# BUTSpeechFIT/DiariZen

Measured on AMD Instinct MI355X. Metric: audio-seconds/s (RTF) for wavlm-large-s80 pipeline, 16 kHz mono, higher is better.
Workload: dtype f32 (operands split into 2 fp16 terms with exact power-of-two scaling = 22 significant bits, 3 fp16 MFMA products, fp32 accumulate: the error-corrected '3xFP16/3xTF32' scheme; kernels without an fp16 variant use the 3-term bf16 split)

## Files before the change

### diarizen_amd/csrc/gemm.hip

```cpp
#include <cstdio>
#include <cstdlib>

#include "common.h"
#include "gemm_epilogue.h"

namespace {

template <bool LOWP>
struct Frag {
  using type = f32x4;
};
template <>
struct Frag<true> {
  using type = bf16x8;
};

__device__ __forceinline__ uint4 pack_bf16x8(const float4& a, const float4& b) {
  bf16x8 v;
  v[0] = (__bf16)a.x; v[1] = (__bf16)a.y; v[2] = (__bf16)a.z; v[3] = (__bf16)a.w;
  v[4] = (__bf16)b.x; v[5] = (__bf16)b.y; v[6] = (__bf16)b.z; v[7] = (__bf16)b.w;
  return *reinterpret_cast<uint4*>(&v);
}

template <int BM, int BN, int WGM, int WGN, bool LOWP>
// ... 88 lines not shown
        rw[i] = make_uint4(0u, 0u, 0u, 0u);
      }
    }
  };

  auto store_tile = [&](int buf) {
    unsigned char* sA = smem + buf * BUF;
    unsigned char* sW = sA + BM * 128;
#pragma unroll
    for (int i = 0; i < ACH; ++i) {
      const int r = r0 + 32 * i;
      const int off = r * 128 + ((c ^ ((r >> 1) & 7)) << 4);
      if constexpr (LOWP)
        *reinterpret_cast<uint4*>(sA + off) = pack_bf16x8(ra[i][0], ra[i][1]);
      else
        *reinterpret_cast<float4*>(sA + off) = ra[i][0];
    }
#pragma unroll
    for (int i = 0; i < WCH; ++i) {
      const int r = r0 + 32 * i;
      const int off = r * 128 + ((c ^ ((r >> 1) & 7)) << 4);
      *reinterpret_cast<uint4*>(sW + off) = rw[i];
    }
  };

  f32x4 acc[MI][NI];
#pragma unroll
  for (int i = 0; i < MI; ++i)
#pragma unroll
    for (int j = 0; j < NI; ++j) acc[i][j] = (f32x4){0.f, 0.f, 0.f, 0.f};

  const int lr = lane & 15;
  const int lq = lane >> 4;

  auto compute = [&](int buf) {
    const unsigned char* sA = smem + buf * BUF;
    const unsigned char* sW = sA + BM * 128;
#pragma unroll
    for (int kb = 0; kb < 2; ++kb) {
      frag_t af[MI], bf[NI];
#pragma unroll
      for (int i = 0; i < MI; ++i) {
        const int row = wm * TM + i * 16 + lr;
        const int slot = (kb * 4 + lq) ^ ((row >> 1) & 7);
        af[i] = *reinterpret_cast<const frag_t*>(sA + row * 128 + (slot << 4));
      }
#pragma unroll
      for (int j = 0; j < NI; ++j) {
        const int row = wn * TN + j * 16 + lr;
        const int slot = (kb * 4 + lq) ^ ((row >> 1) & 7);
        bf[j] = *reinterpret_cast<const frag_t*>(sW + row * 128 + (slot << 4));
      }
      if constexpr (LOWP) {
#pragma unroll
        for (int i = 0; i < MI; ++i)
#pragma unroll
          for (int j = 0; j < NI; ++j)
            acc[i][j] = __builtin_amdgcn_mfma_f32_16x16x32_bf16(bf[j], af[i], acc[i][j], 0, 0, 0);
      } else {
#pragma unroll
        for (int s = 0; s < 4; ++s)
#pragma unroll
          for (int i = 0; i < MI; ++i)
#pragma unroll
            for (int j = 0; j < NI; ++j)
              acc[i][j] = __builtin_amdgcn_mfma_f32_16x16x4f32(bf[j][s], af[i][s], acc[i][j], 0, 0, 0);
      }
    }
  };

  const int nk = (d.K + BK - 1) / BK;
  load_tile(0);
  store_tile(0);
  __syncthreads();
  for (int kt = 0; kt < nk; ++kt) {
    const bool more = kt + 1 < nk;
    if (more) load_tile((kt + 1) * BK);
    compute(kt & 1);
    if (more) store_tile((kt + 1) & 1);
    __syncthreads();
  }

  gemm_epilogue<BM, BN, TM, TN, MI, NI>(d, acc, tm, tn, wm, wn, lr, lq, cz, bz, z0);
}

template <int BM, int BN, int WGM, int WGN>
__global__ __launch_bounds__(256) void gemm_glds_kernel(const dzn_gemm_desc d) {
  static_assert(WGM * WGN == 4, "4 wavefronts per workgroup");
  constexpr int BK = 32;
  constexpr int TM = BM / WGM, TN = BN / WGN;
  constexpr int MI = TM / 16, NI = TN / 16;
  constexpr int ACH = BM / 32, WCH = BN / 32;
  constexpr int BUF = (BM + BN) * 128;
  extern __shared__ __attribute__((aligned(16))) unsigned char smem[];

  const int tid = threadIdx.x, lane = tid & 63, wave = tid >> 6;
  const int wm = wave / WGN, wn = wave % WGN;
  const int tilesN = (d.N + BN - 1) / BN;
  int t;
  {
    const int nwg = gridDim.x, bid = blockIdx.x;
    const int q = nwg >> 3, r = nwg & 7, xcd = bid & 7, idx = bid >> 3;
    t = (xcd < r ? xcd * (q + 1) : r * (q + 1) + (xcd - r) * q) + idx;
  }
  const int tm = t / tilesN, tn = t % tilesN;
  const int z = blockIdx.y;
  int z0 = z / d.zdiv;
  const int z1 = z - z0 * d.zdiv;
  if (d.z_list) {
    if (z0 >= d.z_count[0]) return;
    z0 = d.z_list[z0];
  }
  const float* __restrict__ A = d.A + z0 * d.a_z0 + z1 * d.a_z1;
  const float* __restrict__ W = d.W + z0 * d.w_z0 + z1 * d.w_z1;
  const int64_t cz = z0 * d.c_z0 + z1 * d.c_z1;
  const int64_t bz = z0 * d.b_z0 + z1 * d.b_z1;

  const int r0 = tid >> 3;
  const int csw = (tid & 7) ^ ((r0 >> 1) & 7);
  int64_t abase[ACH], wbase[WCH];
#pragma unroll
  for (int i = 0; i < ACH; ++i) {
    int m = tm * BM + r0 + 32 * i;
    m = m < d.M ? m : d.M - 1;
    abase[i] = (d.a_rowoff ? (int64_t)d.a_rowoff[m] : (int64_t)m * d.lda) + csw * 4;
  }
#pragma unroll
  for (int i = 0; i < WCH; ++i) {
    int n = tn * BN + r0 + 32 * i;
    n = n < d.N ? n : d.N - 1;
    wbase[i] = (int64_t)n * d.ldw + csw * 4;
  }

  auto issue = [&](int k0, int buf) {
    const int ch = k0 / d.kc;
    const int64_t koff = (int64_t)ch * d.ldk + (k0 - ch * d.kc);
    unsigned char* sA = smem + buf * BUF + wave * 1024;
    unsigned char* sW = smem + buf * BUF + BM * 128 + wave * 1024;
#pragma unroll
    for (int i = 0; i < ACH; ++i)
      __builtin_amdgcn_global_load_lds(
          (const __attribute__((address_space(1))) void*)(A + abase[i] + koff),
          (__attribute__((address_space(3))) void*)(sA + i * 4096), 16, 0, 0);
#pragma unroll
    for (int i = 0; i < WCH; ++i)
      __builtin_amdgcn_global_load_lds(
          (const __attribute__((address_space(1))) void*)(W + wbase[i] + k0),
          (__attribute__((address_space(3))) void*)(sW + i * 4096), 16, 0, 0);
  };

  f32x4 acc[MI][NI];
#pragma unroll
  for (int i = 0; i < MI; ++i)
#pragma unroll
    for (int j = 0; j < NI; ++j) acc[i][j] = (f32x4){0.f, 0.f, 0.f, 0.f};
  const int lr = lane & 15, lq = lane >> 4;

  auto read_frags = [&](int buf, int kb, f32x4 (&af)[MI], f32x4 (&bf)[NI]) {
    const unsigned char* sA = smem + buf * BUF;
    const unsigned char* sW = sA + BM * 128;
#pragma unroll
    for (int i = 0; i < MI; ++i) {
      const int row = wm * TM + i * 16 + lr;
      const int slot = (kb * 4 + lq) ^ ((row >> 1) & 7);
      af[i] = *reinterpret_cast<const f32x4*>(sA + row * 128 + (slot << 4));
    }
#pragma unroll
    for (int j = 0; j < NI; ++j) {
      const int row = wn * TN + j * 16 + lr;
      const int slot = (kb * 4 + lq) ^ ((row >> 1) & 7);
      bf[j] = *reinterpret_cast<const f32x4*>(sW + row * 128 + (slot << 4));
    }
  };
  auto mma = [&](const f32x4 (&af)[MI], const f32x4 (&bf)[NI]) {
#pragma unroll
    for (int s = 0; s < 4; ++s)
#pragma unroll
      for (int i = 0; i < MI; ++i)
#pragma unroll
        for (int j = 0; j < NI; ++j)
          acc[i][j] = __builtin_amdgcn_mfma_f32_16x16x4f32(bf[j][s], af[i][s], acc[i][j], 0, 0, 0);
  };

  const int nk = d.K / BK;
  f32x4 a0[MI], b0[NI], a1[MI], b1[NI];
  issue(0, 0);
  __syncthreads();
  read_frags(0, 0, a0, b0);
  for (int kt = 0; kt < nk; ++kt) {
    const int buf = kt & 1;
    const bool more = kt + 1 < nk;
    if (more) issue((kt + 1) * BK, buf ^ 1);
    read_frags(buf, 1, a1, b1);
    __builtin_amdgcn_sched_barrier(0);
    mma(a0, b0);
    __builtin_amdgcn_sched_barrier(0);
    __syncthreads();
    if (more) read_frags(buf ^ 1, 0, a0, b0);
    __builtin_amdgcn_sched_barrier(0);
    mma(a1, b1);
    __builtin_amdgcn_sched_barrier(0);
  }
  gemm_epilogue<BM, BN, TM, TN, MI, NI>(d, acc, tm, tn, wm, wn, lr, lq, cz, bz, z0);
}

template <int BM, int BN, int WGM, int WGN, bool LOWP>
int launch_cfg(const dzn_gemm_desc& d, hipStream_t s) {
  const int tilesM = (d.M + BM - 1) / BM, tilesN = (d.N + BN - 1) / BN;
  static const int lds_pad = getenv("DZN_GEMM_LDS_PAD") ? atoi(getenv("DZN_GEMM_LDS_PAD")) : 0;
  const size_t lds = 2 * (BM + BN) * 128 + lds_pad;
  auto kern = gemm_kernel<BM, BN, WGM, WGN, LOWP>;
  static unsigned long long attr_mask = 0;
  if (first_use_on_device(attr_mask)) {
    (void)hipFuncSetAttribute(reinterpret_cast<const void*>(kern),
                        hipFuncAttributeMaxDynamicSharedMemorySize, 160 * 1024);
    if constexpr (!LOWP)
      (void)hipFuncSetAttribute(reinterpret_cast<const void*>(gemm_glds_kernel<BM, BN, WGM, WGN>),
                                hipFuncAttributeMaxDynamicSharedMemorySize, 160 * 1024);
  }
  static const bool no_glds = getenv("DZN_NO_GLDS") != nullptr;
  const bool use_glds = !LOWP && !no_glds && (d.K % 32 == 0) && (d.kc % 32 == 0);
  dim3 grid(tilesM * tilesN, d.nz > 0 ? d.nz : 1, 1);
  int pid = -1;
  if (prof_enabled()) {
    char cls[64];
    static const bool by_shape = getenv("DZN_PROFILE_SHAPES") != nullptr;
    if (by_shape)
      snprintf(cls, sizeof(cls), "gemm_%s_%dx%d M%d N%d K%d z%d", LOWP ? "bf16" : "f32", BM, BN, d.M, d.N,
               d.K, d.nz);
    else
      snprintf(cls, sizeof(cls), "gemm_%s_%dx%d", LOWP ? "bf16" : "f32", BM, BN);
    const double fl = d.alg_flops > 0 ? d.alg_flops * d.nz : 2.0 * d.M * d.N * d.K * d.nz;
    pid = prof_begin(s, cls, fl, gemm_alg_bytes(d, LOWP ? 2 : 4));
  }
  if constexpr (!LOWP) {
    if (use_glds)
      hipLaunchKernelGGL((gemm_glds_kernel<BM, BN, WGM, WGN>), grid, dim3(256), lds, s, d);
    else
      hipLaunchKernelGGL(kern, grid, dim3(256), lds, s, d);
  } else {
    hipLaunchKernelGGL(kern, grid, dim3(256), lds, s, d);
  }
  prof_end(pid, s);
  if (hipGetLastError() != hipSuccess) return DZN_E_HIP;
  if (d.stat_partial && d.stat_final)
    return launch_stats_finalize(d.stat_partial, d.M, ((d.N + BN - 1) / BN) * WGN, d.stat_C, d.stat_eps, d.stat_final, s);
  return DZN_OK;
}

template <bool LOWP>
int launch_prec(const dzn_gemm_desc& d, hipStream_t s) {
  static const char* force = getenv("DZN_GEMM_CFG");
  if (force) {
    if (!strcmp(force, "128x32")) return launch_cfg<128, 32, 4, 1, LOWP>(d, s);
    if (!strcmp(force, "256x32")) return launch_cfg<256, 32, 4, 1, LOWP>(d, s);
    if (!strcmp(force, "256x64")) return launch_cfg<256, 64, 4, 1, LOWP>(d, s);
    if (!strcmp(force, "128x64")) return launch_cfg<128, 64, 2, 2, LOWP>(d, s);
    if (!strcmp(force, "64x64")) return launch_cfg<64, 64, 2, 2, LOWP>(d, s);
    if (!strcmp(force, "128x128")) return launch_cfg<128, 128, 2, 2, LOWP>(d, s);
  }
  if (d.N <= 32) return launch_cfg<256, 32, 4, 1, LOWP>(d, s);
  if (d.N <= 64) return launch_cfg<128, 64, 2, 2, LOWP>(d, s);
  if (d.K <= 512 && (d.N % 64) == 0) return launch_cfg<128, 64, 2, 2, LOWP>(d, s);
  const int cand[4] = {192, 160, 128, 96};
  int best = 128, best_cols = 1 << 30;
  for (int c : cand) {
    const int cols = (d.N + c - 1) / c * c;
    if (cols < best_cols) { best_cols = cols; best = c; }
  }
  switch (best) {
    case 192: return launch_cfg<128, 192, 2, 2, LOWP>(d, s);
    case 160: return launch_cfg<128, 160, 2, 2, LOWP>(d, s);
    case 96: return launch_cfg<128, 96, 2, 2, LOWP>(d, s);
    default: return launch_cfg<128, 128, 2, 2, LOWP>(d, s);
  }
}

}

int launch_gemm(const dzn_gemm_desc& din, hipStream_t s) {
  dzn_gemm_desc d = din;
  if (d.M <= 0 || d.N <= 0) return DZN_OK;
  if (d.K <= 0 || (d.K & 7)) return DZN_E_INVALID;
  if (d.kc <= 0) { d.kc = d.K; d.ldk = 0; }
  if (d.kc & 7) return DZN_E_INVALID;
  if (d.zdiv <= 0) d.zdiv = 1;
  if (d.nz <= 0) d.nz = 1;
  if (d.alpha == 0.f) d.alpha = 1.f;
  if (d.precision == DZN_PREC_BF16) {
    if (!d.W16) return DZN_E_INVALID;
#ifdef DZN_TUNING
    if (d.a_bf16) return launch_gemm_lowp(d, s);
#else
    if (d.a_bf16) return DZN_E_INVALID;
#endif
    if (d.c_bf16 || d.r_bf16) return DZN_E_INVALID;
    return launch_prec<true>(d, s);
  }
  if (!d.W) return DZN_E_INVALID;
  if (d.kv_planes) {
    const bool ok = d.kv_scale && d.precision == DZN_PREC_F32_H2 && d.W3 && d.W2h && d.col_scale && d.a_amax && !(d.K & 31) &&
                    !(d.kc & 31) && d.ldw == d.K && !d.a_split3 && d.nz == 1 && !d.c_rowoff && d.kv_col0 >= 0 &&
                    d.kv_col0 < d.N && !(d.kv_col0 & 63) && !(d.N & 63) && d.kv_ld == d.N - d.kv_col0 &&
                    !(d.kv_plane_stride & 3) && d.N > 32 && !getenv("DZN_GEMM_CFG") && !getenv("DZN_NO_H2");
    if (!ok) return DZN_E_INVALID;
  }
  if (d.ln_centered && !(d.precision == DZN_PREC_F16 && d.W3 && !(d.K & 31) && !(d.kc & 31) && d.ldw == d.K && !d.a_split3))
    return DZN_E_INVALID;
  if (d.a_split3) return prec_is_split(d.precision) ? launch_gemm_split_pre(d, s) : DZN_E_INVALID;
  if (prec_is_split(d.precision) && d.W3 && !(d.K & 31) && !(d.kc & 31) && d.ldw == d.K)
    return launch_gemm_split(d, s);
  return launch_prec<false>(d, s);
}

extern "C" int dzn_op_gemm(const dzn_gemm_desc* d, void* stream) {
  if (!d || !d->A || !d->C) return DZN_E_INVALID;
  return launch_gemm(*d, reinterpret_cast<hipStream_t>(stream));
}
```

### diarizen_amd/csrc/gemm_split.hip

```cpp
#include <cmath>
#include <cstdio>
#include <cstdlib>
#include <type_traits>

#include "checked.h"
#include "common.h"
#include "gemm_epilogue.h"
#include "split.h"

DZN_CHECKED_TU(gemm_split)

namespace {

__device__ __forceinline__ int wswz(int row) { return (0x78 >> (2 * ((row >> 2) & 3))) & 3; }

template <int N>
__device__ __forceinline__ void wait_vm_lgkm0() {
  static_assert(N >= 0 && N < 64, "vmcnt range");
  __builtin_amdgcn_s_waitcnt((N & 0xF) | ((N >> 4) << 14) | (0x7 << 4));
}

template <int BM, int BN, int WGM, int WGN, int S, int NP, int OCC = 1, int ABL = 0, bool RPF = false>
__global__ __launch_bounds__(WGM * WGN * 64, OCC) void gemm_split_kernel(const dzn_gemm_desc d, const int ngroups) {
  constexpr int NW = WGM * WGN;
  constexpr int BK = 32;
  constexpr int TM = BM / WGM, TN = BN / WGN;
  constexpr int MI = TM / 16, NI = TN / 16, MH = MI / 2;
  constexpr int RB = NW * 1024;
  constexpr int ACH = BM * 128 / RB;
  constexpr int WROWS = NW * 16;
  constexpr int WR = (BN + WROWS - 1) / WROWS;
  constexpr int SP = NP == 3 ? 3 : 2;
  constexpr int ABYTES = BM * 128, WPLANE = BN * 64, BUF = ABYTES + NP * WPLANE;
  constexpr int LPT = ACH + NP * WR;
  constexpr bool WPART = BN % WROWS != 0;
  static_assert(BM * 128 % RB == 0, "A tile must be whole rounds");
  static_assert(MI % 2 == 0, "two row halves per wavefront tile");
  static_assert(S >= 2 && (S - 1) * LPT < 64, "vmcnt range");
  extern __shared__ __attribute__((aligned(16))) unsigned char smem[];

  const int tid = threadIdx.x, lane = tid & 63;
  const int wave = __builtin_amdgcn_readfirstlane(tid >> 6);
  const int wm = wave / WGN, wn = wave % WGN;
  const int tilesN = (d.N + BN - 1) / BN;
  int t;
  {
    const int nwg = gridDim.x, bid = blockIdx.x;
    const int q = nwg >> 3, r = nwg & 7, xcd = bid & 7, idx = bid >> 3;
    t = (xcd < r ? xcd * (q + 1) : r * (q + 1) + (xcd - r) * q) + idx;
  }
  int tm, tn;
  if (ngroups <= 1) {
    tm = t / tilesN;
    tn = t % tilesN;
  } else {
    const int tilesM_ = (int)gridDim.x / tilesN;
    const int base = tilesN / ngroups, rem = tilesN % ngroups;
    int g = 0, cg = base + (rem > 0), cs = 0, r = t;
    while (r >= tilesM_ * cg) {
      r -= tilesM_ * cg;
      cs += cg;
      ++g;
      cg = base + (g < rem);
    }
    tm = r / cg;
    tn = cs + r - tm * cg;
  }
  const int z = blockIdx.y;
  int z0 = z / d.zdiv;
  const int z1 = z - z0 * d.zdiv;
  if (d.z_list) {
    if (z0 >= d.z_count[0]) return;
    z0 = d.z_list[z0];
  }
  const float* __restrict__ A = d.A + z0 * d.a_z0 + z1 * d.a_z1;
  const u16* __restrict__ W3 =
      reinterpret_cast<const u16*>(NP == 3 ? d.W3 : d.W2h) + SP * (z0 * d.w_z0 + z1 * d.w_z1);
  float a_scale[MI], row_inv[MI];
#pragma unroll
  for (int i = 0; i < MI; ++i) a_scale[i] = row_inv[i] = 1.f;
  if constexpr (NP <= 2) {
#pragma unroll
    for (int i = 0; i < MI; ++i) {
      int m = tm * BM + wm * TM + i * 16 + (lane & 15);
      m = m < d.M ? m : d.M - 1;
      const int unit = d.amax_unit > 0 ? m / d.amax_unit : z0;
      DZN_CHECK(d.amax_count <= 0 || (unit >= 0 && unit < d.amax_count), 0x101, unit);
      h2_scale(d.a_amax[unit], a_scale[i], row_inv[i]);
    }
  }
  float a_mean[MI];
#pragma unroll
  for (int i = 0; i < MI; ++i) a_mean[i] = 0.f;
  if constexpr (NP == 1) {
    if (d.ln_centered && d.ln_stats) {
#pragma unroll
      for (int i = 0; i < MI; ++i) {
        int m = tm * BM + wm * TM + i * 16 + (lane & 15);
        m = m < d.M ? m : d.M - 1;
        a_mean[i] = d.ln_stats[2 * (int64_t)m];
        a_scale[i] *= 0.5f;
        row_inv[i] *= 2.f;
      }
    }
  }
  const int64_t cz = z0 * d.c_z0 + z1 * d.c_z1;
  const int64_t bz = z0 * d.b_z0 + z1 * d.b_z1;

  const int r0 = tid >> 3;
  const int csw = (tid & 7) ^ ((r0 >> 1) & 7);
  const float* aptr[ACH];
#pragma unroll
  for (int i = 0; i < ACH; ++i) {
    int m = tm * BM + r0 + 8 * NW * i;
    m = m < d.M ? m : d.M - 1;
    aptr[i] = A + (d.a_rowoff ? (int64_t)d.a_rowoff[m] : (int64_t)m * d.lda) + csw * 4;
  }
  const bool wfull = !WPART || (WR - 1) * WROWS + wave * 16 < BN;
  const int wr0 = wave * 16 + (lane >> 2);
  const int wsw = (lane & 3) ^ wswz(wr0);
  const u16* wptr[WR];
#pragma unroll
  for (int i = 0; i < WR; ++i) {
    int n = tn * BN + wr0 + WROWS * i;
    n = n < d.N ? n : d.N - 1;
    wptr[i] = W3 + (int64_t)n * SP * d.ldw + wsw * 8;
  }

  int ik = 0, irem = 0;
  int64_t ikoff = 0;
  auto issue = [&](int stage) {
    unsigned char* sA = smem + stage * BUF + wave * 1024;
    unsigned char* sW = smem + stage * BUF + ABYTES + wave * 1024;
    DZN_CHECK(stage >= 0 && stage < S && ik < d.K, 0x102, stage);
    DZN_CHECK(wave * 1024 + (ACH - 1) * RB + 1024 <= ABYTES, 0x103, wave);
    DZN_CHECK(!wfull || wave * 1024 + (WR - 1) * RB + 1024 <= WPLANE, 0x104, wave);
#pragma unroll
    for (int i = 0; i < ACH; ++i)
      __builtin_amdgcn_global_load_lds((const __attribute__((address_space(1))) void*)(aptr[i] + ikoff),
                                       (__attribute__((address_space(3))) void*)(sA + i * RB), 16, 0, 0);
#pragma unroll
    for (int p = 0; p < NP; ++p)
#pragma unroll
      for (int i = 0; i < WR; ++i)
        if (i + 1 < WR || wfull)
          __builtin_amdgcn_global_load_lds(
              (const __attribute__((address_space(1))) void*)(wptr[i] + SP * ik + p * 32),
              (__attribute__((address_space(3))) void*)(sW + p * WPLANE + i * RB), 16, 0, 0);
    ik += BK;
    irem += BK;
    ikoff += BK;
    if (irem == d.kc) { irem = 0; ikoff += d.ldk - d.kc; }
  };

  f32x4 acc[MI][NI];
#pragma unroll
  for (int i = 0; i < MI; ++i)
#pragma unroll
    for (int j = 0; j < NI; ++j) acc[i][j] = (f32x4){0.f, 0.f, 0.f, 0.f};
  const int lr = lane & 15, lq = lane >> 4;
  f32x4 rpre[RPF ? MI : 1][RPF ? NI : 1];
  bool use_rpre = false;
  if constexpr (RPF) {
    use_rpre = d.R != nullptr && gemm_epilogue_vec(d, cz, bz);
    if (use_rpre) gemm_prefetch_residual<BM, BN, TM, TN, MI, NI>(d, rpre, tm, tn, wm, wn, lr, lq, cz);
  }

  int woff[NI], aoff0[MI], aoff1[MI];
#pragma unroll
  for (int j = 0; j < NI; ++j) {
    const int row = wn * TN + j * 16 + lr;
    woff[j] = ABYTES + row * 64 + ((lq ^ wswz(row)) << 4);
  }
#pragma unroll
  for (int i = 0; i < MI; ++i) {
    const int row = wm * TM + i * 16 + lr;
    const int sw = (row >> 1) & 7;
    aoff0[i] = row * 128 + ((lq ^ sw) << 4);
    aoff1[i] = row * 128 + (((4 + lq) ^ sw) << 4);
  }
#pragma unroll
  for (int j = 0; j < NI; ++j) DZN_CHECK(woff[j] >= ABYTES && woff[j] + (NP - 1) * WPLANE + 16 <= BUF, 0x105, woff[j]);
#pragma unroll
  for (int i = 0; i < MI; ++i) DZN_CHECK(aoff0[i] + 16 <= ABYTES && aoff1[i] + 16 <= ABYTES, 0x106, aoff1[i]);
  DZN_CHECK(tm * BM < d.M && tn * BN < d.N, 0x107, t);
  auto read_w = [&](int stage, u32x4 (&wf)[NI][NP]) {
    const unsigned char* base = smem + stage * BUF;
#pragma unroll
    for (int j = 0; j < NI; ++j)
#pragma unroll
      for (int p = 0; p < NP; ++p) wf[j][p] = *reinterpret_cast<const u32x4*>(base + p * WPLANE + woff[j]);
  };
  auto read_a = [&](int stage, f32x4 (&ar)[MI][2]) {
    const unsigned char* base = smem + stage * BUF;
#pragma unroll
    for (int i = 0; i < MI; ++i) {
      ar[i][0] = *reinterpret_cast<const f32x4*>(base + aoff0[i]);
      ar[i][1] = *reinterpret_cast<const f32x4*>(base + aoff1[i]);
    }
  };
  auto mma = [&](int i, const u32x4 (&wf)[NI][NP], const u32x4 (&af)[NP]) {
    if constexpr (ABL == 2) {
#pragma unroll
      for (int j = 0; j < NI; ++j) acc[i][j][0] += __uint_as_float(wf[j][0][0] ^ af[0][0]);
    } else if constexpr (NP == 3) {
      constexpr int PW[6] = {2, 0, 1, 1, 0, 0}, PA[6] = {0, 2, 1, 0, 1, 0};
#pragma unroll
      for (int t = 0; t < 6; ++t)
#pragma unroll
        for (int j = 0; j < NI; ++j) acc[i][j] = mfma_np<NP>(wf[j][PW[t]], af[PA[t]], acc[i][j]);
    } else if constexpr (NP == 2) {
      constexpr int PW[3] = {1, 0, 0}, PA[3] = {0, 1, 0};
#pragma unroll
      for (int t = 0; t < 3; ++t)
#pragma unroll
        for (int j = 0; j < NI; ++j) acc[i][j] = mfma_np<NP>(wf[j][PW[t]], af[PA[t]], acc[i][j]);
    } else {
#pragma unroll
      for (int j = 0; j < NI; ++j) acc[i][j] = mfma_np<NP>(wf[j][0], af[0], acc[i][j]);
    }
  };
  auto split = [&](const f32x4 (&a)[2], u32x4 (&af)[NP], float sc, float mu = 0.f) {
    if constexpr (ABL == 1) {
#pragma unroll
      for (int p = 0; p < NP; ++p) af[p] = __builtin_bit_cast(u32x4, a[p & 1]);
    } else if constexpr (NP == 3) {
      bf16x8 h_, m_, l_;
      split8(a[0], a[1], h_, m_, l_);
      af[0] = __builtin_bit_cast(u32x4, h_);
      af[1] = __builtin_bit_cast(u32x4, m_);
      af[2] = __builtin_bit_cast(u32x4, l_);
    } else if constexpr (NP == 2) {
      split8_h2(a[0], a[1], sc, af[0], af[1]);
    } else {
      cvt8_h1(a[0] - mu, a[1] - mu, sc, af[0]);
    }
  };

  const int nk = d.K / BK;
#pragma unroll
  for (int s = 0; s < S; ++s)
    if (s < nk) issue(s);
  auto wait_tiles = [&](auto tiles) {
    constexpr int T = decltype(tiles)::value;
    if (wfull) wait_vm_lgkm0<T * LPT>();
    else wait_vm_lgkm0<T * (LPT - NP)>();
  };
  if (nk >= S) wait_tiles(std::integral_constant<int, S - 1>{});
  else wait_vm_lgkm0<0>();
  __builtin_amdgcn_s_barrier();
  u32x4 wfa[NI][NP], wfb[NI][NP];
  f32x4 ar[MI][2];
  read_w(0, wfa);
  read_a(0, ar);
  if constexpr (ABL == 5) read_w(0, wfb);
  int stage = 0;

  auto step = [&](int kt, const u32x4 (&wc)[NI][NP], u32x4 (&wn_)[NI][NP]) {
    const bool more = kt + 1 < nk;
#pragma unroll
    for (int i = 0; i < MH; ++i) {
      u32x4 af[NP];
      split(ar[i], af, a_scale[i], a_mean[i]);
      mma(i, wc, af);
    }
    u32x4 af2[MI - MH][NP];
#pragma unroll
    for (int i = MH; i < MI; ++i) split(ar[i], af2[i - MH], a_scale[i], a_mean[i]);
    const int nstage = stage + 1 == S ? 0 : stage + 1;
    __builtin_amdgcn_sched_barrier(0);
    if (more) {
      if (kt + S <= nk) wait_tiles(std::integral_constant<int, S - 2>{});
      else wait_vm_lgkm0<0>();
      if constexpr (ABL != 4) __builtin_amdgcn_s_barrier();
      if constexpr (ABL != 3)
        if (kt + S < nk) issue(stage);
      if constexpr (ABL != 5) {
        read_w(nstage, wn_);
        read_a(nstage, ar);
      }
    }
    __builtin_amdgcn_sched_barrier(0);
#pragma unroll
    for (int i = MH; i < MI; ++i) mma(i, wc, af2[i - MH]);
    stage = nstage;
  };
  for (int kt = 0; kt < nk; kt += 2) {
    step(kt, wfa, wfb);
    if (kt + 1 < nk) step(kt + 1, wfb, wfa);
  }
  if constexpr (true) {
    __syncthreads();
    if constexpr (RPF) {
      if (use_rpre) {
        gemm_epilogue<BM, BN, TM, TN, MI, NI, true>(d, acc, tm, tn, wm, wn, lr, lq, cz, bz, z0, row_inv, NP <= 2 ? d.col_scale : nullptr,
                                                    reinterpret_cast<float*>(smem) + wave * 3 * TN, rpre);
        return;
      }
    }
    gemm_epilogue<BM, BN, TM, TN, MI, NI, true>(d, acc, tm, tn, wm, wn, lr, lq, cz, bz, z0, row_inv, NP <= 2 ? d.col_scale : nullptr,
                                                reinterpret_cast<float*>(smem) + wave * 3 * TN);
  } else {
    gemm_epilogue<BM, BN, TM, TN, MI, NI>(d, acc, tm, tn, wm, wn, lr, lq, cz, bz, z0, row_inv, NP <= 2 ? d.col_scale : nullptr);
  }
}

#ifdef DZN_TUNING
typedef float f32x16 __attribute__((ext_vector_type(16)));

template <int BM, int BN, int WGM, int WGN, int S, int NP, int OCC = 1, int PRIO = 0>
__global__ __launch_bounds__(WGM * WGN * 64, OCC) void gemm_split32_kernel(const dzn_gemm_desc d) {
  static_assert(NP == 1 || NP == 2, "fp16 forms only");
  constexpr int NW = WGM * WGN;
  constexpr int BK = 32;
  constexpr int TM = BM / WGM, TN = BN / WGN;
  constexpr int MI = TM / 32, NJ = TN / 32;
  constexpr int RB = NW * 1024;
  constexpr int ACH = BM * 128 / RB;
  constexpr int WROWS = NW * 16;
  constexpr int WR = (BN + WROWS - 1) / WROWS;
  constexpr int ABYTES = BM * 128, WPLANE = BN * 64, BUF = ABYTES + NP * WPLANE;
  constexpr int LPT = ACH + NP * WR;
  constexpr bool WPART = BN % WROWS != 0;
  static_assert(BM * 128 % RB == 0 && TM % 32 == 0 && TN % 32 == 0, "tile geometry");
  static_assert(S >= 2 && (S - 1) * LPT < 64, "vmcnt range");
  extern __shared__ __attribute__((aligned(16))) unsigned char smem[];

  const int tid = threadIdx.x, lane = tid & 63;
  const int wave = __builtin_amdgcn_readfirstlane(tid >> 6);
  const int wm = wave / WGN, wn = wave % WGN;
  const int tilesN = (d.N + BN - 1) / BN;
  int t;
  {
    const int nwg = gridDim.x, bid = blockIdx.x;
    const int q = nwg >> 3, r = nwg & 7, xcd = bid & 7, idx = bid >> 3;
    t = (xcd < r ? xcd * (q + 1) : r * (q + 1) + (xcd - r) * q) + idx;
  }
  const int tm = t / tilesN, tn = t % tilesN;
  const int z = blockIdx.y;
  int z0 = z / d.zdiv;
  const int z1 = z - z0 * d.zdiv;
  if (d.z_list) {
    if (z0 >= d.z_count[0]) return;
    z0 = d.z_list[z0];
  }
  const float* __restrict__ A = d.A + z0 * d.a_z0 + z1 * d.a_z1;
  const u16* __restrict__ W2 = reinterpret_cast<const u16*>(d.W2h) + 2 * (z0 * d.w_z0 + z1 * d.w_z1);
  const int l31 = lane & 31, lh = lane >> 5;
  float a_scale[MI], row_inv[MI];
#pragma unroll
  for (int i = 0; i < MI; ++i) {
    int m = tm * BM + wm * TM + i * 32 + l31;
    m = m < d.M ? m : d.M - 1;
    h2_scale(d.a_amax[d.amax_unit > 0 ? m / d.amax_unit : z0], a_scale[i], row_inv[i]);
  }
  const int64_t cz = z0 * d.c_z0 + z1 * d.c_z1;
  const int64_t bz = z0 * d.b_z0 + z1 * d.b_z1;

  const int r0 = tid >> 3;
  const int csw = (tid & 7) ^ ((r0 >> 1) & 7);
  const float* aptr[ACH];
#pragma unroll
  for (int i = 0; i < ACH; ++i) {
    int m = tm * BM + r0 + 8 * NW * i;
    m = m < d.M ? m : d.M - 1;
    aptr[i] = A + (d.a_rowoff ? (int64_t)d.a_rowoff[m] : (int64_t)m * d.lda) + csw * 4;
  }
  const bool wfull = !WPART || (WR - 1) * WROWS + wave * 16 < BN;
  const int wr0 = wave * 16 + (lane >> 2);
  const int wsw = (lane & 3) ^ wswz(wr0);
  const u16* wptr[WR];
#pragma unroll
  for (int i = 0; i < WR; ++i) {
    int n = tn * BN + wr0 + WROWS * i;
    n = n < d.N ? n : d.N - 1;
    wptr[i] = W2 + (int64_t)n * 2 * d.ldw + wsw * 8;
  }
  int ik = 0, irem = 0;
  int64_t ikoff = 0;
  auto issue = [&](int stage) {
    unsigned char* sA = smem + stage * BUF + wave * 1024;
    unsigned char* sW = smem + stage * BUF + ABYTES + wave * 1024;
#pragma unroll
    for (int i = 0; i < ACH; ++i)
      __builtin_amdgcn_global_load_lds((const __attribute__((address_space(1))) void*)(aptr[i] + ikoff),
                                       (__attribute__((address_space(3))) void*)(sA + i * RB), 16, 0, 0);
#pragma unroll
    for (int p = 0; p < NP; ++p)
#pragma unroll
      for (int i = 0; i < WR; ++i)
        if (i + 1 < WR || wfull)
          __builtin_amdgcn_global_load_lds(
              (const __attribute__((address_space(1))) void*)(wptr[i] + 2 * ik + p * 32),
              (__attribute__((address_space(3))) void*)(sW + p * WPLANE + i * RB), 16, 0, 0);
    ik += BK;
    irem += BK;
    ikoff += BK;
    if (irem == d.kc) { irem = 0; ikoff += d.ldk - d.kc; }
  };

  f32x16 acc[MI][NJ];
#pragma unroll
  for (int i = 0; i < MI; ++i)
#pragma unroll
    for (int j = 0; j < NJ; ++j)
#pragma unroll
      for (int e = 0; e < 16; ++e) acc[i][j][e] = 0.f;

  int woff[NJ][2], aoff0[MI][2], aoff1[MI][2];
#pragma unroll
  for (int j = 0; j < NJ; ++j) {
    const int row = wn * TN + j * 32 + l31;
#pragma unroll
    for (int kh = 0; kh < 2; ++kh) woff[j][kh] = ABYTES + row * 64 + (((2 * kh + lh) ^ wswz(row)) << 4);
  }
#pragma unroll
  for (int i = 0; i < MI; ++i) {
    const int row = wm * TM + i * 32 + l31;
    const int sw = (row >> 1) & 7;
#pragma unroll
    for (int kh = 0; kh < 2; ++kh) {
      const int c = 2 * kh + lh;
      aoff0[i][kh] = row * 128 + ((c ^ sw) << 4);
      aoff1[i][kh] = row * 128 + (((4 + c) ^ sw) << 4);
    }
  }
  auto read_w = [&](int stage, u32x4 (&wf)[NJ][2][NP]) {
    const unsigned char* base = smem + stage * BUF;
#pragma unroll
    for (int j = 0; j < NJ; ++j)
#pragma unroll
      for (int kh = 0; kh < 2; ++kh)
#pragma unroll
        for (int p = 0; p < NP; ++p) wf[j][kh][p] = *reinterpret_cast<const u32x4*>(base + p * WPLANE + woff[j][kh]);
  };
  auto read_a = [&](int stage, f32x4 (&ar)[MI][2][2]) {
    const unsigned char* base = smem + stage * BUF;
#pragma unroll
    for (int i = 0; i < MI; ++i)
#pragma unroll
      for (int kh = 0; kh < 2; ++kh) {
        ar[i][kh][0] = *reinterpret_cast<const f32x4*>(base + aoff0[i][kh]);
        ar[i][kh][1] = *reinterpret_cast<const f32x4*>(base + aoff1[i][kh]);
      }
  };
  auto mfma32 = [&](const u32x4& a, const u32x4& b, f32x16 c) {
    return __builtin_amdgcn_mfma_f32_32x32x16_f16(__builtin_bit_cast(f16x8, a), __builtin_bit_cast(f16x8, b), c, 0, 0, 0);
  };
  auto mma = [&](int i, int kh, const u32x4 (&wf)[NJ][2][NP], const u32x4 (&af)[NP]) {
    if constexpr (PRIO) __builtin_amdgcn_s_setprio(1);
    if constexpr (NP == 2) {
      constexpr int PW[3] = {1, 0, 0}, PA[3] = {0, 1, 0};
#pragma unroll
      for (int t = 0; t < 3; ++t)
#pragma unroll
        for (int j = 0; j < NJ; ++j) acc[i][j] = mfma32(wf[j][kh][PW[t]], af[PA[t]], acc[i][j]);
    } else {
#pragma unroll
      for (int j = 0; j < NJ; ++j) acc[i][j] = mfma32(wf[j][kh][0], af[0], acc[i][j]);
    }
    if constexpr (PRIO) __builtin_amdgcn_s_setprio(0);
  };
  auto split = [&](const f32x4 (&a)[2], u32x4 (&af)[NP], float sc) {
    if constexpr (NP == 2) split8_h2(a[0], a[1], sc, af[0], af[1]);
    else cvt8_h1(a[0], a[1], sc, af[0]);
  };

  const int nk = d.K / BK;
#pragma unroll
  for (int s = 0; s < S; ++s)
    if (s < nk) issue(s);
  auto wait_tiles = [&](auto tiles) {
    constexpr int T = decltype(tiles)::value;
    if (wfull) wait_vm_lgkm0<T * LPT>();
    else wait_vm_lgkm0<T * (LPT - NP)>();
  };
  if (nk >= S) wait_tiles(std::integral_constant<int, S - 1>{});
  else wait_vm_lgkm0<0>();
  __builtin_amdgcn_s_barrier();
  u32x4 wfa[NJ][2][NP], wfb[NJ][2][NP];
  f32x4 ar[MI][2][2];
  read_w(0, wfa);
  read_a(0, ar);
  int stage = 0;

  auto step = [&](int kt, const u32x4 (&wc)[NJ][2][NP], u32x4 (&wn_)[NJ][2][NP]) {
    const bool more = kt + 1 < nk;
#pragma unroll
    for (int i = 0; i < MI; ++i) {
      u32x4 af[NP];
      split(ar[i][0], af, a_scale[i]);
      mma(i, 0, wc, af);
    }
    u32x4 af2[MI][NP];
#pragma unroll
    for (int i = 0; i < MI; ++i) split(ar[i][1], af2[i], a_scale[i]);
    const int nstage = stage + 1 == S ? 0 : stage + 1;
    __builtin_amdgcn_sched_barrier(0);
    if (more) {
      if (kt + S <= nk) wait_tiles(std::integral_constant<int, S - 2>{});
      else wait_vm_lgkm0<0>();
      __builtin_amdgcn_s_barrier();
      if (kt + S < nk) issue(stage);
      read_w(nstage, wn_);
      read_a(nstage, ar);
    }
    __builtin_amdgcn_sched_barrier(0);
#pragma unroll
    for (int i = 0; i < MI; ++i) mma(i, 1, wc, af2[i]);
    stage = nstage;
  };
  for (int kt = 0; kt < nk; kt += 2) {
    step(kt, wfa, wfb);
    if (kt + 1 < nk) step(kt + 1, wfb, wfa);
  }
  __syncthreads();
  f32x4 accv[MI][4 * NJ];
#pragma unroll
  for (int i = 0; i < MI; ++i)
#pragma unroll
    for (int j = 0; j < NJ; ++j)
#pragma unroll
      for (int g = 0; g < 4; ++g)
#pragma unroll
        for (int e = 0; e < 4; ++e) accv[i][4 * j + g][e] = acc[i][j][4 * g + e];
  gemm_epilogue<BM, BN, TM, TN, MI, 4 * NJ, true, 32, 8>(d, accv, tm, tn, wm, wn, l31, lh, cz, bz, z0, row_inv, d.col_scale,
                                                       reinterpret_cast<float*>(smem) + wave * 3 * TN);
}

template <int BM, int BN, int WGM, int WGN, int S, int NP, int OCC = 1, int PRIO = 0>
int launch_split32_cfg(const dzn_gemm_desc& d, hipStream_t s) {
  const int tilesM = (d.M + BM - 1) / BM, tilesN = (d.N + BN - 1) / BN;
  const size_t lds = (size_t)S * (BM * 128 + NP * BN * 64);
  auto kern = gemm_split32_kernel<BM, BN, WGM, WGN, S, NP, OCC, PRIO>;
  static unsigned long long attr_mask = 0;
  if (first_use_on_device(attr_mask))
    (void)hipFuncSetAttribute(reinterpret_cast<const void*>(kern), hipFuncAttributeMaxDynamicSharedMemorySize, 160 * 1024);
  dim3 grid(tilesM * tilesN, d.nz > 0 ? d.nz : 1, 1);
  int pid = -1;
  if (prof_enabled()) {
    char cls[64];
    static const bool by_shape = getenv("DZN_PROFILE_SHAPES") != nullptr;
    if (by_shape)
      snprintf(cls, sizeof(cls), "gemm_%s_%dx%d M%d N%d K%d z%d", NP == 2 ? "f32h" : "f16", BM, BN, d.M, d.N, d.K, d.nz);
    else
      snprintf(cls, sizeof(cls), "gemm_%s_%dx%d", NP == 2 ? "f32h" : "f16", BM, BN);
    const double fl = d.alg_flops > 0 ? d.alg_flops * d.nz : 2.0 * d.M * d.N * d.K * d.nz;
    pid = prof_begin(s, cls, fl, gemm_alg_bytes(d, NP * 2));
  }
  hipLaunchKernelGGL(kern, grid, dim3(WGM * WGN * 64), lds, s, d);
  prof_end(pid, s);
  if (hipGetLastError() != hipSuccess) return DZN_E_HIP;
  if (d.stat_partial && d.stat_final)
    return launch_stats_finalize(d.stat_partial, d.M, tilesN * WGN, d.stat_C, d.stat_eps, d.stat_final, s);
  return DZN_OK;
}

#endif

int choose_column_groups(const dzn_gemm_desc& d, int tilesM, int tilesN, int BM, int NP) {
  static const char* env = getenv("DZN_GEMM_NGROUPS");
  static const bool automatic = env && !strcmp(env, "auto");
  static const int forced = env && !automatic ? atoi(env) : 0;
  if (tilesN < 2 || d.w_z0 || d.w_z1 || (!automatic && forced <= 1)) return 1;
  if (forced > 0) return forced < tilesN ? (forced > 8 ? 8 : forced) : tilesN > 8 ? 8 : tilesN;
  if ((d.nz > 1) || (int64_t)tilesM * tilesN < 1024) return 1;
  const double W = (double)d.N * d.K * 2.0 * NP;
  const double a_cols = d.a_rowoff ? (double)d.kc : (d.lda > 0 && d.lda < d.K ? (double)d.lda : (double)d.K);
  const double A = (double)d.M * a_cols * 4.0;
  auto miss = [](double bytes) {
    static const double mb[] = {0.5, 1.0, 2.0, 4.0, 8.0, 12.0}, f[] = {0.02, 0.055, 0.12, 0.27, 0.69, 1.0};
    const double x = bytes / (1024.0 * 1024.0);
    if (x <= mb[0]) return f[0] * x / mb[0];
    for (int i = 1; i < 6; ++i)
      if (x <= mb[i]) return f[i - 1] + (f[i] - f[i - 1]) * (log2(x) - log2(mb[i - 1])) / (log2(mb[i]) - log2(mb[i - 1]));
    return 1.0;
  };
  int best = 1;
  const double r1 = A + tilesM * W * miss(W);
  double rbest = r1;
  for (int G = 2; G <= 8 && G <= tilesN; G *= 2) {
    const double r = G * A + tilesM * W * miss(W / G);
    if (r < rbest) { rbest = r; best = G; }
  }
  (void)BM;
  return rbest < 0.95 * r1 ? best : 1;
}

template <int BM, int BN, int WGM, int WGN, int S, int NP, int OCC = 1, int ABL = 0, bool RPF = false>
int launch_split_cfg(const dzn_gemm_desc& d, hipStream_t s) {
  const int tilesM = (d.M + BM - 1) / BM, tilesN = (d.N + BN - 1) / BN;
  const size_t lds = (size_t)S * (BM * 128 + NP * BN * 64);
  auto kern = gemm_split_kernel<BM, BN, WGM, WGN, S, NP, OCC, ABL, RPF>;
  static unsigned long long attr_mask = 0;
  if (first_use_on_device(attr_mask)) {
    (void)hipFuncSetAttribute(reinterpret_cast<const void*>(kern), hipFuncAttributeMaxDynamicSharedMemorySize,
                              160 * 1024);
  }
  dim3 grid(tilesM * tilesN, d.nz > 0 ? d.nz : 1, 1);
  int pid = -1;
  if (prof_enabled()) {
    char cls[64];
    static const bool by_shape = getenv("DZN_PROFILE_SHAPES") != nullptr;
    if (by_shape)
      snprintf(cls, sizeof(cls), "gemm_%s_%dx%d M%d N%d K%d z%d", NP == 3 ? "f32s" : NP == 2 ? "f32h" : "f16", BM, BN, d.M,
               d.N, d.K, d.nz);
    else
      snprintf(cls, sizeof(cls), "gemm_%s_%dx%d%s", NP == 3 ? "f32s" : NP == 2 ? "f32h" : "f16", BM, BN, RPF ? "_rpf" : "");
    const double fl = d.alg_flops > 0 ? d.alg_flops * d.nz : 2.0 * d.M * d.N * d.K * d.nz;
    pid = prof_begin(s, cls, fl, gemm_alg_bytes(d, NP * 2));
  }
  hipLaunchKernelGGL(kern, grid, dim3(WGM * WGN * 64), lds, s, d, choose_column_groups(d, tilesM, tilesN, BM, NP));
  prof_end(pid, s);
  if (hipGetLastError() != hipSuccess) return DZN_E_HIP;
  if (d.stat_partial && d.stat_final)
    return launch_stats_finalize(d.stat_partial, d.M, tilesN * WGN, d.stat_C, d.stat_eps, d.stat_final, s);
  return DZN_OK;
}

__global__ __launch_bounds__(256) void split_weights_kernel(const float* __restrict__ W, int64_t rows, int K,
                                                            int64_t ldw, u16* __restrict__ W3) {
  const int64_t n = rows * K;
  for (int64_t i = (int64_t)blockIdx.x * 256 + threadIdx.x; i < n; i += (int64_t)gridDim.x * 256) {
    const int64_t r = i / K;
    const int k = (int)(i - r * K);
    const float x = W[r * ldw + k];
    const __bf16 h = (__bf16)x;
    const float r1 = x - (float)h;
    const __bf16 m = (__bf16)r1;
    const float r2 = r1 - (float)m;
    const __bf16 l = (__bf16)r2;
    const int kk = k & 31;
    const int pos = 8 * ((kk & 15) >> 2) + (kk & 3) + 4 * (kk >> 4);
    u16* o = W3 + r * 3 * K + (int64_t)(k >> 5) * 96 + pos;
    o[0] = *reinterpret_cast<const u16*>(&h);
    o[32] = *reinterpret_cast<const u16*>(&m);
    o[64] = *reinterpret_cast<const u16*>(&l);
  }
}

char g_force_buf[32] = {0};
bool g_force_init = false;
const char* g_force_cfg() {
  if (!g_force_init) {
    const char* e = getenv("DZN_GEMM_CFG");
    if (e) snprintf(g_force_buf, sizeof(g_force_buf), "%s", e);
    g_force_init = true;
  }
  return g_force_buf[0] ? g_force_buf : nullptr;
}

template <int NP>
int launch_gemm_split_np(const dzn_gemm_desc& d, hipStream_t s) {
  const char* force = g_force_cfg();
  if (force) {
    if (!strcmp(force, "128x64")) return launch_split_cfg<128, 64, 4, 1, 2, NP, NP <= 2 ? 3 : 2>(d, s);
    if (!strcmp(force, "128x80")) return launch_split_cfg<128, 80, 4, 1, 2, NP, 2>(d, s);
    if (!strcmp(force, "128x32")) return launch_split_cfg<128, 32, 4, 1, 2, NP>(d, s);
    if constexpr (NP == 3) {
      if (!strcmp(force, "128x128")) return launch_split_cfg<128, 128, 2, 2, 2, NP, 2>(d, s);
    } else {
      if (!strcmp(force, "128x128w4")) return launch_split_cfg<128, 128, 4, 1, 2, NP, 2>(d, s);
    }
    if constexpr (NP == 1) {
      if (!strcmp(force, "256x128w8s3")) return launch_split_cfg<256, 128, 8, 1, 3, NP, 2>(d, s);
    }
#ifdef DZN_TUNING
    if constexpr (NP <= 2) {
      if (!strcmp(force, "m32_128x128")) return launch_split32_cfg<128, 128, 4, 1, 2, NP, 2>(d, s);
      if (!strcmp(force, "m32_128x64")) return launch_split32_cfg<128, 64, 4, 1, 2, NP, 3>(d, s);
    }
    if (!strcmp(force, "256x128")) return launch_split_cfg<256, 128, 4, 2, 2, NP>(d, s);
    if constexpr (NP != 3) {
      if (!strcmp(force, "128x128")) return launch_split_cfg<128, 128, 2, 2, 2, NP>(d, s);
    }
    if constexpr (NP <= 2) {
      if (!strcmp(force, "m32_128x128p")) return launch_split32_cfg<128, 128, 4, 1, 2, NP, 2, 1>(d, s);
      if (!strcmp(force, "m32_128x128w22")) return launch_split32_cfg<128, 128, 2, 2, 2, NP, 2>(d, s);
      if (!strcmp(force, "m32_256x128")) return launch_split32_cfg<256, 128, 4, 2, 2, NP, 1>(d, s);
      if (!strcmp(force, "m32_256x128w8")) return launch_split32_cfg<256, 128, 8, 1, 2, NP, 1>(d, s);
      if (!strcmp(force, "m32_128x64p")) return launch_split32_cfg<128, 64, 4, 1, 2, NP, 3, 1>(d, s);
      if (!strcmp(force, "256x128s3")) return launch_split_cfg<256, 128, 4, 2, 3, NP>(d, s);
      if (!strcmp(force, "256x128w8s3")) return launch_split_cfg<256, 128, 8, 1, 3, NP, 2>(d, s);
      if (!strcmp(force, "128x64s3")) return launch_split_cfg<128, 64, 4, 1, 3, NP>(d, s);
      if (!strcmp(force, "256x64s3")) return launch_split_cfg<256, 64, 8, 1, 3, NP>(d, s);
      if (!strcmp(force, "abl1")) return launch_split_cfg<128, 128, 4, 1, 2, NP, 2, 1>(d, s);
      if (!strcmp(force, "abl2")) return launch_split_cfg<128, 128, 4, 1, 2, NP, 2, 2>(d, s);
      if (!strcmp(force, "abl3")) return launch_split_cfg<128, 128, 4, 1, 2, NP, 2, 3>(d, s);
      if (!strcmp(force, "abl4")) return launch_split_cfg<128, 128, 4, 1, 2, NP, 2, 4>(d, s);
      if (!strcmp(force, "abl5")) return launch_split_cfg<128, 128, 4, 1, 2, NP, 2, 5>(d, s);
    }
#endif
  }
#ifdef DZN_TUNING
  static const int m32 = getenv("DZN_GEMM_M32") ? atoi(getenv("DZN_GEMM_M32")) : 0;
#else
  constexpr int m32 = 0;
#endif
  constexpr int OCC64 = NP <= 2 ? 3 : 2;
  if (d.N <= 32) return launch_split_cfg<128, 32, 4, 1, 2, NP>(d, s);
#ifdef DZN_TUNING
  if constexpr (NP <= 2) {
    if ((m32 & 2) && d.N > 32 && (d.N <= 64 || d.K <= 512)) return launch_split32_cfg<128, 64, 4, 1, 2, NP, 3>(d, s);
  }
#endif
  if constexpr (NP == 2) {
    static const int rpf = getenv("DZN_GEMM_RPF") ? atoi(getenv("DZN_GEMM_RPF")) : 0;
    if (rpf && d.R && d.N > 64 && d.K <= 512) {
      return launch_split_cfg<128, 64, 4, 1, 2, NP, 2, 0, true>(d, s);
    }
  }
  if (d.N <= 64 || d.K <= 512) return launch_split_cfg<128, 64, 4, 1, 2, NP, OCC64>(d, s);
  const int cols128 = (d.N + 127) / 128 * 128, cols64 = (d.N + 63) / 64 * 64;
  if ((int64_t)((d.M + 127) / 128) * (cols128 / 128) * (d.nz > 0 ? d.nz : 1) < 448)
    return launch_split_cfg<128, 64, 4, 1, 2, NP, OCC64>(d, s);
  if (d.N % 80 == 0 && d.N < cols64 && d.N * 9 < cols128 * 8) return launch_split_cfg<128, 80, 4, 1, 2, NP, 2>(d, s);
  if (cols64 * 9 < cols128 * 8) return launch_split_cfg<128, 64, 4, 1, 2, NP, OCC64>(d, s);
  if constexpr (NP == 1) return launch_split_cfg<256, 128, 8, 1, 3, NP, 2>(d, s);
  if constexpr (NP == 2) {
#ifdef DZN_TUNING
    if (m32 & 1) return launch_split32_cfg<128, 128, 4, 1, 2, NP, 2>(d, s);
#endif
    return launch_split_cfg<128, 128, 4, 1, 2, NP, 2>(d, s);
  }
  return launch_split_cfg<128, 128, 2, 2, 2, NP, 2>(d, s);
}

__global__ __launch_bounds__(256) void split_weights_h2_kernel(const float* __restrict__ W, int64_t rows, int K,
                                                               int64_t ldw, u16* __restrict__ W2, float* __restrict__ col_scale) {
  const int lane = threadIdx.x & 63;
  const int64_t r = (int64_t)blockIdx.x * 4 + (threadIdx.x >> 6);
  if (r >= rows) return;
  float m = 0.f;
  for (int k = lane; k < K; k += 64) m = fmaxf(m, fabsf(W[r * ldw + k]));
  m = wave_max(m);
  float sc, inv;
  h2_scale(m, sc, inv);
  if (lane == 0) col_scale[r] = inv;
  for (int k = lane; k < K; k += 64) {
    const float x = W[r * ldw + k] * sc;
    const _Float16 h = (_Float16)x;
    const _Float16 l = (_Float16)(x - (float)h);
    const int kk = k & 31;
    const int pos = 8 * ((kk & 15) >> 2) + (kk & 3) + 4 * (kk >> 4);
    u16* o = W2 + r * 2 * K + (int64_t)(k >> 5) * 64 + pos;
    o[0] = __builtin_bit_cast(u16, h);
    o[32] = __builtin_bit_cast(u16, l);
  }
}

}

int launch_gemm_split(const dzn_gemm_desc& d, hipStream_t s) {
  if ((d.K & 31) || (d.kc & 31) || d.ldw != d.K) return DZN_E_INVALID;
  static const bool no_h2 = getenv("DZN_NO_H2") != nullptr;
  if (d.precision == DZN_PREC_F16 && d.Wmx && d.col_scale_mx && d.a_amax && !d.w_z0 && !d.w_z1 && !no_h2)
    return d.ln_centered ? DZN_E_INVALID : launch_gemm_mx(d, s);
  if (prec_is_h2(d.precision) && d.W2h && d.col_scale && d.a_amax && !d.w_z0 && !d.w_z1 && !no_h2) {
    if (d.precision == DZN_PREC_F16) return launch_gemm_split_np<1>(d, s);
    return d.ln_centered ? DZN_E_INVALID : launch_gemm_split_np<2>(d, s);
  }
  if (!d.W3 || d.ln_centered) return DZN_E_INVALID;
  return launch_gemm_split_np<3>(d, s);
}

extern "C" int dzn_op_set_gemm_cfg(const char* cfg) {
  g_force_init = true;
  snprintf(g_force_buf, sizeof(g_force_buf), "%s", cfg && strcmp(cfg, "auto") ? cfg : "");
  return DZN_OK;
}

int launch_split_weights_h2(const float* W, int64_t rows, int K, int64_t ldw, void* W2, float* col_scale, hipStream_t s) {
  if (rows <= 0) return DZN_OK;
  if (K <= 0 || (K & 31)) return DZN_E_INVALID;
  hipLaunchKernelGGL(split_weights_h2_kernel, dim3((unsigned)cdiv64(rows, 4)), dim3(256), 0, s, W, rows, K, ldw,
                     static_cast<u16*>(W2), col_scale);
  return hipGetLastError() == hipSuccess ? DZN_OK : DZN_E_HIP;
}

extern "C" int dzn_op_split_weights_h2(const float* W, int64_t rows, int32_t K, int64_t ldw, void* W2, float* col_scale,
                                       void* stream) {
  if (!W || !W2 || !col_scale) return DZN_E_INVALID;
  return launch_split_weights_h2(W, rows, K, ldw, W2, col_scale, reinterpret_cast<hipStream_t>(stream));
}

int launch_split_weights(const float* W, int64_t rows, int K, int64_t ldw, void* W3, hipStream_t s) {
  if (rows <= 0) return DZN_OK;
  if (K <= 0 || (K & 31)) return DZN_E_INVALID;
  int64_t g = cdiv64(rows * K, 256);
  g = g > 8192 ? 8192 : g;
  hipLaunchKernelGGL(split_weights_kernel, dim3((unsigned)g), dim3(256), 0, s, W, rows, K, ldw,
                     static_cast<u16*>(W3));
  return hipGetLastError() == hipSuccess ? DZN_OK : DZN_E_HIP;
}

extern "C" int dzn_op_split_weights(const float* W, int64_t rows, int32_t K, int64_t ldw, void* W3, void* stream) {
  if (!W || !W3) return DZN_E_INVALID;
  return launch_split_weights(W, rows, K, ldw, W3, reinterpret_cast<hipStream_t>(stream));
}
```

Baseline: 1753.

## Skip MFMA work for out-of-range column blocks in split GEMM warps

Each wavefront counts how many of its 16-column blocks fall inside N (and whether its rows are inside M) and dispatches to a compile-time specialization that only reads weights and issues MFMAs for the live blocks. Fully dead waves still take part in the barriers and load issue. Because padded N no longer costs compute, the heuristic that fell back to 64-wide tiles when 128-padding wasted columns is removed, so such shapes now use 128-wide tiles. Guards for the kv_planes path are moved into the launchers. The cost is more template instantiations, larger code and more register pressure.

```diff
diff --git a/diarizen_amd/csrc/gemm.hip b/diarizen_amd/csrc/gemm.hip
--- a/diarizen_amd/csrc/gemm.hip
+++ b/diarizen_amd/csrc/gemm.hip
@@ -414,7 +414,7 @@
     const bool ok = d.kv_scale && d.precision == DZN_PREC_F32_H2 && d.W3 && d.W2h && d.col_scale && d.a_amax && !(d.K & 31) &&
                     !(d.kc & 31) && d.ldw == d.K && !d.a_split3 && d.nz == 1 && !d.c_rowoff && d.kv_col0 >= 0 &&
                     d.kv_col0 < d.N && !(d.kv_col0 & 63) && !(d.N & 63) && d.kv_ld == d.N - d.kv_col0 &&
-                    !(d.kv_plane_stride & 3) && d.N > 32 && !getenv("DZN_GEMM_CFG") && !getenv("DZN_NO_H2");
+                    !(d.kv_plane_stride & 3) && d.N > 32 && !getenv("DZN_NO_H2");
     if (!ok) return DZN_E_INVALID;
   }
   if (d.ln_centered && !(d.precision == DZN_PREC_F16 && d.W3 && !(d.K & 31) && !(d.kc & 31) && d.ldw == d.K && !d.a_split3))
diff --git a/diarizen_amd/csrc/gemm_split.hip b/diarizen_amd/csrc/gemm_split.hip
--- a/diarizen_amd/csrc/gemm_split.hip
+++ b/diarizen_amd/csrc/gemm_split.hip
@@ -18,6 +18,12 @@
 __device__ __forceinline__ void wait_vm_lgkm0() {
   static_assert(N >= 0 && N < 64, "vmcnt range");
   __builtin_amdgcn_s_waitcnt((N & 0xF) | ((N >> 4) << 14) | (0x7 << 4));
+}
+
+template <int J, class F>
+__device__ __forceinline__ void with_live_blocks(int nj, F&& f) {
+  if (nj == J) f(std::integral_constant<int, J>{});
+  else if constexpr (J > 0) with_live_blocks<J - 1>(nj, f);
 }
 
 template <int BM, int BN, int WGM, int WGN, int S, int NP, int OCC = 1, int ABL = 0, bool RPF = false>
@@ -184,10 +190,11 @@
 #pragma unroll
   for (int i = 0; i < MI; ++i) DZN_CHECK(aoff0[i] + 16 <= ABYTES && aoff1[i] + 16 <= ABYTES, 0x106, aoff1[i]);
   DZN_CHECK(tm * BM < d.M && tn * BN < d.N, 0x107, t);
-  auto read_w = [&](int stage, u32x4 (&wf)[NI][NP]) {
+  auto read_w = [&](int stage, auto& wf) {
+    constexpr int NJ = std::extent<std::remove_reference_t<decltype(wf)>>::value;
     const unsigned char* base = smem + stage * BUF;
 #pragma unroll
-    for (int j = 0; j < NI; ++j)
+    for (int j = 0; j < NJ; ++j)
 #pragma unroll
       for (int p = 0; p < NP; ++p) wf[j][p] = *reinterpret_cast<const u32x4*>(base + p * WPLANE + woff[j]);
   };
@@ -199,25 +206,26 @@
       ar[i][1] = *reinterpret_cast<const f32x4*>(base + aoff1[i]);
     }
   };
-  auto mma = [&](int i, const u32x4 (&wf)[NI][NP], const u32x4 (&af)[NP]) {
+  auto mma = [&](int i, const auto& wf, const u32x4 (&af)[NP]) {
+    constexpr int NJ = std::extent<std::remove_reference_t<decltype(wf)>>::value;
     if constexpr (ABL == 2) {
 #pragma unroll
-      for (int j = 0; j < NI; ++j) acc[i][j][0] += __uint_as_float(wf[j][0][0] ^ af[0][0]);
+      for (int j = 0; j < NJ; ++j) acc[i][j][0] += __uint_as_float(wf[j][0][0] ^ af[0][0]);
     } else if constexpr (NP == 3) {
       constexpr int PW[6] = {2, 0, 1, 1, 0, 0}, PA[6] = {0, 2, 1, 0, 1, 0};
 #pragma unroll
       for (int t = 0; t < 6; ++t)
 #pragma unroll
-        for (int j = 0; j < NI; ++j) acc[i][j] = mfma_np<NP>(wf[j][PW[t]], af[PA[t]], acc[i][j]);
+        for (int j = 0; j < NJ; ++j) acc[i][j] = mfma_np<NP>(wf[j][PW[t]], af[PA[t]], acc[i][j]);
     } else if constexpr (NP == 2) {
       constexpr int PW[3] = {1, 0, 0}, PA[3] = {0, 1, 0};
 #pragma unroll
       for (int t = 0; t < 3; ++t)
 #pragma unroll
-        for (int j = 0; j < NI; ++j) acc[i][j] = mfma_np<NP>(wf[j][PW[t]], af[PA[t]], acc[i][j]);
+        for (int j = 0; j < NJ; ++j) acc[i][j] = mfma_np<NP>(wf[j][PW[t]], af[PA[t]], acc[i][j]);
     } else {
 #pragma unroll
-      for (int j = 0; j < NI; ++j) acc[i][j] = mfma_np<NP>(wf[j][0], af[0], acc[i][j]);
+      for (int j = 0; j < NJ; ++j) acc[i][j] = mfma_np<NP>(wf[j][0], af[0], acc[i][j]);
     }
   };
   auto split = [&](const f32x4 (&a)[2], u32x4 (&af)[NP], float sc, float mu = 0.f) {
@@ -249,46 +257,59 @@
   if (nk >= S) wait_tiles(std::integral_constant<int, S - 1>{});
   else wait_vm_lgkm0<0>();
   __builtin_amdgcn_s_barrier();
-  u32x4 wfa[NI][NP], wfb[NI][NP];
-  f32x4 ar[MI][2];
-  read_w(0, wfa);
-  read_a(0, ar);
-  if constexpr (ABL == 5) read_w(0, wfb);
-  int stage = 0;
-
-  auto step = [&](int kt, const u32x4 (&wc)[NI][NP], u32x4 (&wn_)[NI][NP]) {
-    const bool more = kt + 1 < nk;
-#pragma unroll
-    for (int i = 0; i < MH; ++i) {
-      u32x4 af[NP];
-      split(ar[i], af, a_scale[i], a_mean[i]);
-      mma(i, wc, af);
-    }
-    u32x4 af2[MI - MH][NP];
-#pragma unroll
-    for (int i = MH; i < MI; ++i) split(ar[i], af2[i - MH], a_scale[i], a_mean[i]);
-    const int nstage = stage + 1 == S ? 0 : stage + 1;
-    __builtin_amdgcn_sched_barrier(0);
-    if (more) {
-      if (kt + S <= nk) wait_tiles(std::integral_constant<int, S - 2>{});
-      else wait_vm_lgkm0<0>();
-      if constexpr (ABL != 4) __builtin_amdgcn_s_barrier();
-      if constexpr (ABL != 3)
-        if (kt + S < nk) issue(stage);
-      if constexpr (ABL != 5) {
-        read_w(nstage, wn_);
-        read_a(nstage, ar);
+  int nj = (d.N - tn * BN - wn * TN + 15) >> 4;
+  nj = nj < 0 ? 0 : nj > NI ? NI : nj;
+  if (tm * BM + wm * TM >= d.M) nj = 0;
+  nj = __builtin_amdgcn_readfirstlane(nj);
+  with_live_blocks<NI>(nj, [&](auto live) {
+    constexpr int NJ = decltype(live)::value;
+    u32x4 wfa[NJ ? NJ : 1][NP], wfb[NJ ? NJ : 1][NP];
+    f32x4 ar[MI][2];
+    if constexpr (NJ > 0) {
+      read_w(0, wfa);
+      read_a(0, ar);
+      if constexpr (ABL == 5) read_w(0, wfb);
+    }
+    int stage = 0;
+
+    auto step = [&](int kt, const auto& wc, auto& wn_) {
+      const bool more = kt + 1 < nk;
+      u32x4 af2[MI - MH][NP];
+      if constexpr (NJ > 0) {
+#pragma unroll
+        for (int i = 0; i < MH; ++i) {
+          u32x4 af[NP];
+          split(ar[i], af, a_scale[i], a_mean[i]);
+          mma(i, wc, af);
+        }
+#pragma unroll
+        for (int i = MH; i < MI; ++i) split(ar[i], af2[i - MH], a_scale[i], a_mean[i]);
       }
-    }
-    __builtin_amdgcn_sched_barrier(0);
-#pragma unroll
-    for (int i = MH; i < MI; ++i) mma(i, wc, af2[i - MH]);
-    stage = nstage;
-  };
-  for (int kt = 0; kt < nk; kt += 2) {
-    step(kt, wfa, wfb);
-    if (kt + 1 < nk) step(kt + 1, wfb, wfa);
-  }
+      const int nstage = stage + 1 == S ? 0 : stage + 1;
+      __builtin_amdgcn_sched_barrier(0);
+      if (more) {
+        if (kt + S <= nk) wait_tiles(std::integral_constant<int, S - 2>{});
+        else wait_vm_lgkm0<0>();
+        if constexpr (ABL != 4) __builtin_amdgcn_s_barrier();
+        if constexpr (ABL != 3)
+          if (kt + S < nk) issue(stage);
+        if constexpr (ABL != 5 && NJ > 0) {
+          read_w(nstage, wn_);
+          read_a(nstage, ar);
+        }
+      }
+      __builtin_amdgcn_sched_barrier(0);
+      if constexpr (NJ > 0) {
+#pragma unroll
+        for (int i = MH; i < MI; ++i) mma(i, wc, af2[i - MH]);
+      }
+      stage = nstage;
+    };
+    for (int kt = 0; kt < nk; kt += 2) {
+      step(kt, wfa, wfb);
+      if (kt + 1 < nk) step(kt + 1, wfb, wfa);
+    }
+  });
   if constexpr (true) {
     __syncthreads();
     if constexpr (RPF) {
@@ -532,6 +553,7 @@
 int launch_split32_cfg(const dzn_gemm_desc& d, hipStream_t s) {
   const int tilesM = (d.M + BM - 1) / BM, tilesN = (d.N + BN - 1) / BN;
   const size_t lds = (size_t)S * (BM * 128 + NP * BN * 64);
+  if (d.kv_planes) return DZN_E_INVALID;
   auto kern = gemm_split32_kernel<BM, BN, WGM, WGN, S, NP, OCC, PRIO>;
   static unsigned long long attr_mask = 0;
   if (first_use_on_device(attr_mask))
@@ -591,6 +613,8 @@
 int launch_split_cfg(const dzn_gemm_desc& d, hipStream_t s) {
   const int tilesM = (d.M + BM - 1) / BM, tilesN = (d.N + BN - 1) / BN;
   const size_t lds = (size_t)S * (BM * 128 + NP * BN * 64);
+  constexpr int MI_ = BM / WGM / 16, NI_ = BN / WGN / 16;
+  if (d.kv_planes && (NP != 2 || epi_chunk(NI_, MI_ * NI_ > 16 ? 4 : 8) % 4 != 0)) return DZN_E_INVALID;
   auto kern = gemm_split_kernel<BM, BN, WGM, WGN, S, NP, OCC, ABL, RPF>;
   static unsigned long long attr_mask = 0;
   if (first_use_on_device(attr_mask)) {
@@ -654,6 +678,7 @@
 int launch_gemm_split_np(const dzn_gemm_desc& d, hipStream_t s) {
   const char* force = g_force_cfg();
   if (force) {
+    if (d.kv_planes) return DZN_E_INVALID;
     if (!strcmp(force, "128x64")) return launch_split_cfg<128, 64, 4, 1, 2, NP, NP <= 2 ? 3 : 2>(d, s);
     if (!strcmp(force, "128x80")) return launch_split_cfg<128, 80, 4, 1, 2, NP, 2>(d, s);
     if (!strcmp(force, "128x32")) return launch_split_cfg<128, 32, 4, 1, 2, NP>(d, s);
@@ -715,7 +740,6 @@
   if ((int64_t)((d.M + 127) / 128) * (cols128 / 128) * (d.nz > 0 ? d.nz : 1) < 448)
     return launch_split_cfg<128, 64, 4, 1, 2, NP, OCC64>(d, s);
   if (d.N % 80 == 0 && d.N < cols64 && d.N * 9 < cols128 * 8) return launch_split_cfg<128, 80, 4, 1, 2, NP, 2>(d, s);
-  if (cols64 * 9 < cols128 * 8) return launch_split_cfg<128, 64, 4, 1, 2, NP, OCC64>(d, s);
   if constexpr (NP == 1) return launch_split_cfg<256, 128, 8, 1, 3, NP, 2>(d, s);
   if constexpr (NP == 2) {
 #ifdef DZN_TUNING
```

Result: no change. 1754, median of 2 (+0.1%).
